# run-house/kubetorch

Hardware: NVIDIA H100
Metric: parallel_map_arg_plus_result_GBps (higher is better)
Workload: dtype f32

## Files before the change

### kubetorch_b200/csrc/ktb_dispatch.cu

```cuda
#include "ktb_common.cuh"

#include <algorithm>
#include <mutex>

namespace ktb {


constexpr int kBcastMax = 15;
constexpr int kBcastThreads = 256;
constexpr int kBcastUnroll = 2;

struct BcastDsts {
  uint8_t* d[kBcastMax];
  int n;
};

__global__ void __launch_bounds__(kBcastThreads)
    bcast_kernel(const uint8_t* src, const __grid_constant__ BcastDsts dsts, size_t n_bytes) {
  constexpr size_t VB = 32;
  constexpr size_t ROW = (size_t)kBcastThreads * VB;
  constexpr size_t TILE = ROW * kBcastUnroll;
  const size_t n_full = n_bytes / TILE;
  for (size_t t = blockIdx.x; t < n_full; t += gridDim.x) {
    const size_t off = t * TILE + (size_t)threadIdx.x * VB;
// ... 37 lines not shown
extern "C" {

int ktb_broadcast(int root, const void* src, void* const* dsts, int n_dst, size_t nbytes,
                  uintptr_t stream) {
  int rc = require_device(root);
  if (rc) return rc;
  KTB_REQUIRE(n_dst >= 0 && n_dst <= kBcastMax, KTB_ERR_ARG, "ktb_broadcast: n_dst %d out of range [0,%d]",
              n_dst, kBcastMax);
  if (nbytes == 0 || n_dst == 0) return KTB_OK;
  KTB_REQUIRE(src && dsts, KTB_ERR_ARG, "ktb_broadcast: null argument");
  BcastDsts b;
  b.n = 0;
  uintptr_t align = (uintptr_t)src;
  for (int k = 0; k < n_dst; ++k) {
    KTB_REQUIRE(dsts[k], KTB_ERR_ARG, "ktb_broadcast: dsts[%d] is null", k);
    if (dsts[k] == src) continue;
    b.d[b.n++] = static_cast<uint8_t*>(dsts[k]);
    align |= (uintptr_t)dsts[k];
  }
  if (b.n == 0) return KTB_OK;
  KTB_GUARD(root);
  const DeviceInfo* di = device_info(root);
  cudaStream_t st = reinterpret_cast<cudaStream_t>(stream);
  if ((align & 31) == 0) {
    size_t tiles = nbytes / ((size_t)kBcastThreads * 32 * kBcastUnroll);
    int grid = (int)std::min<size_t>(std::max<size_t>(tiles, 1), (size_t)di->sm_count * 4);
    bcast_kernel<<<grid, kBcastThreads, 0, st>>>(static_cast<const uint8_t*>(src), b, nbytes);
  } else {
    size_t blocks = (nbytes + 255) / 256;
    int grid = (int)std::min<size_t>(std::max<size_t>(blocks, 1), (size_t)di->sm_count * 8);
    bcast_bytes_kernel<<<grid, 256, 0, st>>>(static_cast<const uint8_t*>(src), b, nbytes);
  }
  KTB_CK(cudaGetLastError());
  return KTB_OK;
}

}

struct CallEvents {
  cudaEvent_t make(int device, int slot) {
    struct Pool {
      cudaEvent_t ev[kMaxDevices][kMaxDevices + 1] = {};
      ~Pool() {}
    };
    static thread_local Pool pool;
    if (device < 0 || device >= kMaxDevices || slot < 0 || slot > kMaxDevices) return nullptr;
    cudaEvent_t& e = pool.ev[device][slot];
    if (!e) {
      DeviceGuard g(device);
      if (!g.ok || cudaEventCreateWithFlags(&e, cudaEventDisableTiming) != cudaSuccess) {
        e = nullptr;
        return nullptr;
      }
    }
    return e;
  }
};

static int check_ranks(const char* who, int n_ranks, const int* devs, int root_rank) {
  KTB_REQUIRE(n_ranks > 0 && n_ranks <= kMaxDevices && devs, KTB_ERR_ARG, "%s: bad n_ranks %d", who, n_ranks);
  KTB_REQUIRE(root_rank >= 0 && root_rank < n_ranks, KTB_ERR_ARG, "%s: root_rank %d out of range", who, root_rank);
  for (int r = 0; r < n_ranks; ++r) {
    int rc = require_device(devs[r]);
    if (rc) return rc;
    if (devs[r] != devs[root_rank]) {
      KTB_REQUIRE(ktb_peer_enabled(devs[r], devs[root_rank]) == 1, KTB_ERR_UNSUPPORTED,
                  "%s: device %d has no peer access to root device %d", who, devs[r], devs[root_rank]);
    }
  }
  return KTB_OK;
}

static cudaStream_t rank_stream(const uintptr_t* streams, const int* devs, int r) {
  return streams ? reinterpret_cast<cudaStream_t>(streams[r]) : device_info(devs[r])->stream_rank;
}

template <class Launch>
static int fork_join(const char* who, size_t n_elems, size_t granule, int n_ranks, const int* devs, int root_rank,
                     const uintptr_t* streams, bool skip_empty, Launch&& launch) {
  const int root_dev = devs[root_rank];
  cudaStream_t root_stream = rank_stream(streams, devs, root_rank);
  CallEvents events;
  cudaEvent_t done[kMaxDevices] = {nullptr};
  cudaEvent_t args_ready = events.make(root_dev, 0);
  KTB_REQUIRE(args_ready, KTB_ERR_CUDA, "%s: cudaEventCreate failed", who);
  {
    KTB_GUARD(root_dev);
    KTB_CK(cudaEventRecord(args_ready, root_stream));
  }
  for (int r = 0; r < n_ranks; ++r) {
    size_t b = 0, e = 0;
    ktb_shard_bounds(n_elems / granule, n_ranks, r, &b, &e);
    b *= granule;
    e *= granule;
    if (skip_empty && e == b) continue;
    const int dev = devs[r];
    KTB_GUARD(dev);
    cudaStream_t st = rank_stream(streams, devs, r);
    const bool is_root = (r == root_rank) || (dev == root_dev && st == root_stream);
    if (!is_root) KTB_CK(cudaStreamWaitEvent(st, args_ready, 0));
    int rc = launch(r, dev, b, e, st);
    if (rc) return rc;
    if (!is_root) {
      done[r] = events.make(dev, 1 + r);
      KTB_REQUIRE(done[r], KTB_ERR_CUDA, "%s: cudaEventCreate failed", who);
      KTB_CK(cudaEventRecord(done[r], st));
    }
  }
  KTB_GUARD(root_dev);
  for (int r = 0; r < n_ranks; ++r)
    if (done[r]) KTB_CK(cudaStreamWaitEvent(root_stream, done[r], 0));
  return KTB_OK;
}

extern "C" {

int ktb_scatter_map_gather(int op, int dtype, const void* src_root, void* dst_root, size_t n_elems,
                           size_t granule, double alpha, double beta, int n_ranks, const int* devs,
                           int root_rank, int variant, const uintptr_t* streams) {
  int rc = check_ranks("ktb_scatter_map_gather", n_ranks, devs, root_rank);
  if (rc) return rc;
  const size_t es = dtype_size(dtype);
  KTB_REQUIRE(es != 0, KTB_ERR_ARG, "ktb_scatter_map_gather: unknown dtype %d", dtype);
  if (n_elems == 0) return KTB_OK;
  KTB_REQUIRE(src_root && dst_root, KTB_ERR_ARG, "ktb_scatter_map_gather: null src/dst");
  KTB_REQUIRE(granule > 0 && n_elems % granule == 0, KTB_ERR_ARG,
              "ktb_scatter_map_gather: n_elems %zu is not a multiple of granule %zu", n_elems, granule);
  const MapParams p = make_params(alpha, beta, dtype);
  return fork_join("ktb_scatter_map_gather", n_elems, granule, n_ranks, devs, root_rank, streams, true,
                   [&](int, int dev, size_t b, size_t e, cudaStream_t st) {
                     return launch_map(dev, op, dtype, static_cast<const uint8_t*>(src_root) + b * es,
                                       static_cast<uint8_t*>(dst_root) + b * es, e - b, p, variant, st);
                   });
}

int ktb_scatter_map_reduce(int op, int dtype, const void* src_root, size_t n_elems, size_t granule,
                           double alpha, double beta, int n_ranks, const int* devs, int root_rank,
                           void* partials_root, void* out_root, void* const* workspaces,
                           const uintptr_t* streams) {
  int rc = check_ranks("ktb_scatter_map_reduce", n_ranks, devs, root_rank);
  if (rc) return rc;
  const size_t es = dtype_size(dtype);
  KTB_REQUIRE(es != 0 && dtype != KTB_U8, KTB_ERR_ARG, "ktb_scatter_map_reduce: dtype %d not reducible", dtype);
  KTB_REQUIRE(partials_root && out_root && workspaces, KTB_ERR_ARG, "ktb_scatter_map_reduce: null argument");
  for (int r = 0; r < n_ranks; ++r)
    KTB_REQUIRE(workspaces[r], KTB_ERR_ARG, "ktb_scatter_map_reduce: workspaces[%d] is null", r);
  KTB_REQUIRE(src_root || n_elems == 0, KTB_ERR_ARG, "ktb_scatter_map_reduce: null src");
  KTB_REQUIRE(granule > 0 && n_elems % granule == 0, KTB_ERR_ARG,
              "ktb_scatter_map_reduce: n_elems %zu is not a multiple of granule %zu", n_elems, granule);
  const MapParams p = make_params(alpha, beta, dtype);
  const size_t acc_size = (dtype == KTB_F32 || dtype == KTB_BF16 || dtype == KTB_F16) ? 4 : 8;
  rc = fork_join("ktb_scatter_map_reduce", n_elems, granule, n_ranks, devs, root_rank, streams, false,
                 [&](int r, int dev, size_t b, size_t e, cudaStream_t st) {
                   return launch_map_reduce(dev, op, dtype, static_cast<const uint8_t*>(src_root) + b * es, e - b, p,
                                            static_cast<uint8_t*>(partials_root) + (size_t)r * acc_size,
                                            workspaces[r], st);
                 });
  if (rc) return rc;
  KTB_GUARD(devs[root_rank]);
  return launch_reduce_partials(devs[root_rank], dtype, partials_root, n_ranks, out_root,
                                rank_stream(streams, devs, root_rank));
}


}
```

### kubetorch_b200/csrc/ktb_map.cu

```cuda
#include "ktb_common.cuh"

#include <algorithm>
#include <atomic>

namespace ktb {

extern int g_red_ctas_per_sm;
extern int g_red_loads;
extern int g_red_fold;
extern int g_seg_large;
extern int g_mlp_chunk_rows;
}
extern int g_mlp_stage_ce;
namespace ktb {
extern std::atomic<int> g_host_zero_copy;
}
extern std::atomic<int> g_push_scatter_ctas_per_sm;
extern std::atomic<int> g_push_slice;
namespace ktb {

static std::atomic<int> g_vec_ctas_per_sm{0};
static std::atomic<int> g_tma_ctas_per_sm{1};
static std::atomic<int> g_tma_cfg{0};
static std::atomic<int> g_auto_variant{KTB_VARIANT_VEC};
static std::atomic<int> g_vec_flavor{2};
static std::atomic<int> g_vec_unroll{4};

constexpr int kVecThreads = 256;
constexpr int kVecUnroll = 4;
constexpr int kVecFlavor = 2;

template <int VB, int FL>
__device__ __forceinline__ void ld_vec(const uint8_t* p, uint32_t (&w)[VB / 4]) {
  static_assert(VB == 16, "sm_90 has no wider per-thread global access than 128 bits");
  if constexpr (FL == 1) {
    asm volatile("ld.global.v4.b32 {%0,%1,%2,%3}, [%4];"
                 : "=r"(w[0]), "=r"(w[1]), "=r"(w[2]), "=r"(w[3])
                 : "l"(p)
                 : "memory");
  } else if constexpr (FL == 2 || FL == 3) {
    ldg128_stream(p, w);
  } else {
    ldg128(p, w);
  }
}
template <int VB, int FL>
__device__ __forceinline__ void st_vec(uint8_t* p, const uint32_t (&w)[VB / 4]) {
  static_assert(VB == 16, "sm_90 has no wider per-thread global access than 128 bits");
  if constexpr (FL == 1) {
    asm volatile("st.global.v4.b32 [%0], {%1,%2,%3,%4};" ::"l"(p), "r"(w[0]), "r"(w[1]), "r"(w[2]), "r"(w[3])
                 : "memory");
  } else if constexpr (FL == 2) {
    stg128_stream(p, w);
  } else {
    stg128(p, w);
  }
}

template <int DT, int OP, int VB, int FL = kVecFlavor, int UNROLL = kVecUnroll>
__global__ void __launch_bounds__(kVecThreads)
    map_vec_kernel(const uint8_t* src, uint8_t* dst, size_t n_bytes, MapParams p) {
  constexpr int NW = VB / 4;
  constexpr int kVecUnroll = UNROLL;
  constexpr size_t TILE = (size_t)kVecThreads * kVecUnroll * VB;
  constexpr size_t ROW = (size_t)kVecThreads * VB;
  const size_t n_full = n_bytes / TILE;

  for (size_t t = blockIdx.x; t < n_full; t += gridDim.x) {
    const size_t off = t * TILE + (size_t)threadIdx.x * VB;
    uint32_t w[kVecUnroll][NW];
#pragma unroll
    for (int j = 0; j < kVecUnroll; ++j) ld_vec<VB, FL>(src + off + j * ROW, w[j]);
#pragma unroll
    for (int j = 0; j < kVecUnroll; ++j) {
      apply_words<DT, OP, NW>(w[j], p);
      st_vec<VB, FL>(dst + off + j * ROW, w[j]);
    }
  }

  if (blockIdx.x == (unsigned)(n_full % gridDim.x)) {
    const size_t base = n_full * TILE;
    const size_t n_vec = (n_bytes - base) / VB;
    for (size_t v = threadIdx.x; v < n_vec; v += kVecThreads) {
      uint32_t w[NW];
      ld_vec<VB, FL>(src + base + v * VB, w);
      apply_words<DT, OP, NW>(w, p);
      st_vec<VB, FL>(dst + base + v * VB, w);
    }
    constexpr size_t ES = (DT == KTB_U8) ? 1 : ((DT == KTB_BF16 || DT == KTB_F16) ? 2 : (DT == KTB_I64 ? 8 : 4));
    const size_t tail = base + n_vec * VB;
    const size_t n_tail = (n_bytes - tail) / ES;
    for (size_t e = threadIdx.x; e < n_tail; e += kVecThreads)
      apply_elem<DT, OP>(src + tail + e * ES, dst + tail + e * ES, p);
  }
}

template <int DT, int OP>
__global__ void __launch_bounds__(256)
    map_scalar_kernel(const uint8_t* src, uint8_t* dst, size_t n_elems, MapParams p) {
  constexpr size_t ES = (DT == KTB_U8) ? 1 : ((DT == KTB_BF16 || DT == KTB_F16) ? 2 : (DT == KTB_I64 ? 8 : 4));
  const size_t stride = (size_t)gridDim.x * blockDim.x;
  for (size_t i = (size_t)blockIdx.x * blockDim.x + threadIdx.x; i < n_elems; i += stride)
    apply_elem<DT, OP>(src + i * ES, dst + i * ES, p);
}

template <int DT, int OP, int STAGES, int STAGE_BYTES, int NT>
__global__ void __launch_bounds__(NT)
    map_tma_kernel(const uint8_t* src, uint8_t* dst, size_t n_bytes, MapParams p) {
  extern __shared__ __align__(128) uint8_t smem[];
  uint8_t* buf = smem;
  uint64_t* full = reinterpret_cast<uint64_t*>(smem + (size_t)STAGES * STAGE_BYTES);
  constexpr bool kCompute = !(OP == KTB_OP_IDENTITY || DT == KTB_U8);
// ... 246 lines not shown
```

### kubetorch_b200/csrc/ktb_mlp.cu

```cuda
#include "ktb_common.cuh"

#include <cuda.h>
#include <algorithm>
#include <atomic>
#include <climits>
#include <cmath>
#include <mutex>

namespace ktb {

constexpr int kMlpBlockM = 128;
constexpr int kMlpBlockK = 64;
constexpr int kMlpWgmmaK = 16;
constexpr int kMlpStages = 4;
constexpr int kMlpConsumers = 256;
constexpr int kMlpThreads = kMlpConsumers + 32;
int g_mlp_chunk_rows = 16896;

__device__ __forceinline__ void tma_load_2d(void* smem_dst, const CUtensorMap* map, int c0, int c1, uint64_t* bar) {
  asm volatile(
      "cp.async.bulk.tensor.2d.shared::cluster.global.mbarrier::complete_tx::bytes [%0], [%1, {%3, %4}], [%2];" ::
          "r"(smem_u32(smem_dst)),
      "l"(map), "r"(smem_u32(bar)), "r"(c0), "r"(c1)
      : "memory");
}
__device__ __forceinline__ void prefetch_tensormap(const CUtensorMap* map) {
  asm volatile("prefetch.tensormap [%0];" ::"l"(map) : "memory");
}
__device__ __forceinline__ void mbar_arrive(uint64_t* bar) {
  asm volatile("mbarrier.arrive.shared::cta.b64 _, [%0];" ::"r"(smem_u32(bar)) : "memory");
}
__device__ __forceinline__ void wgmma_fence() { asm volatile("wgmma.fence.sync.aligned;" ::: "memory"); }
__device__ __forceinline__ void wgmma_commit() { asm volatile("wgmma.commit_group.sync.aligned;" ::: "memory"); }
__device__ __forceinline__ void wgmma_wait_all() { asm volatile("wgmma.wait_group.sync.aligned 0;" ::: "memory"); }

__device__ __forceinline__ uint64_t make_smem_desc_sw128(const void* smem_tile) {
  const uint32_t addr = smem_u32(smem_tile);
  uint64_t d = 0;
  d |= (uint64_t)((addr & 0x3FFFFu) >> 4);
  d |= (uint64_t)1 << 16;
  d |= (uint64_t)(1024u >> 4) << 32;
  d |= (uint64_t)1 << 62;
  return d;
}

template <int N>
struct Wgmma;
template <>
struct Wgmma<256> {
  __device__ __forceinline__ static void mma(float (&d)[128], uint64_t adesc, uint64_t bdesc, uint32_t scale_d) {
    asm volatile(
        "{\n"
        ".reg .pred p;\n"
        "setp.ne.b32 p, %130, 0;\n"
        "wgmma.mma_async.sync.aligned.m64n256k16.f32.bf16.bf16 "
        "{%0,%1,%2,%3,%4,%5,%6,%7,%8,%9,%10,%11,%12,%13,%14,%15,%16,%17,%18,%19,%20,%21,%22,%23,%24,%25,%26,%27,%28,%29,%30,%31,%32,%33,%34,%35,%36,%37,%38,%39,%40,%41,%42,%43,%44,%45,%46,%47,%48,%49,%50,%51,%52,%53,%54,%55,%56,%57,%58,%59,%60,%61,%62,%63,%64,%65,%66,%67,%68,%69,%70,%71,%72,%73,%74,%75,%76,%77,%78,%79,%80,%81,%82,%83,%84,%85,%86,%87,%88,%89,%90,%91,%92,%93,%94,%95,%96,%97,%98,%99,%100,%101,%102,%103,%104,%105,%106,%107,%108,%109,%110,%111,%112,%113,%114,%115,%116,%117,%118,%119,%120,%121,%122,%123,%124,%125,%126,%127}, "
        "%128, %129, p, 1, 1, 0, 0;\n"
        "}\n"
        : "+f"(d[0]), "+f"(d[1]), "+f"(d[2]), "+f"(d[3]), "+f"(d[4]), "+f"(d[5]), "+f"(d[6]), "+f"(d[7]), "+f"(d[8]), "+f"(d[9]), "+f"(d[10]), "+f"(d[11]), "+f"(d[12]), "+f"(d[13]), "+f"(d[14]), "+f"(d[15]), "+f"(d[16]), "+f"(d[17]), "+f"(d[18]), "+f"(d[19]), "+f"(d[20]), "+f"(d[21]), "+f"(d[22]), "+f"(d[23]), "+f"(d[24]), "+f"(d[25]), "+f"(d[26]), "+f"(d[27]), "+f"(d[28]), "+f"(d[29]), "+f"(d[30]), "+f"(d[31]), "+f"(d[32]), "+f"(d[33]), "+f"(d[34]), "+f"(d[35]), "+f"(d[36]), "+f"(d[37]), "+f"(d[38]), "+f"(d[39]), "+f"(d[40]), "+f"(d[41]), "+f"(d[42]), "+f"(d[43]), "+f"(d[44]), "+f"(d[45]), "+f"(d[46]), "+f"(d[47]), "+f"(d[48]), "+f"(d[49]), "+f"(d[50]), "+f"(d[51]), "+f"(d[52]), "+f"(d[53]), "+f"(d[54]), "+f"(d[55]), "+f"(d[56]), "+f"(d[57]), "+f"(d[58]), "+f"(d[59]), "+f"(d[60]), "+f"(d[61]), "+f"(d[62]), "+f"(d[63]), "+f"(d[64]), "+f"(d[65]), "+f"(d[66]), "+f"(d[67]), "+f"(d[68]), "+f"(d[69]), "+f"(d[70]), "+f"(d[71]), "+f"(d[72]), "+f"(d[73]), "+f"(d[74]), "+f"(d[75]), "+f"(d[76]), "+f"(d[77]), "+f"(d[78]), "+f"(d[79]), "+f"(d[80]), "+f"(d[81]), "+f"(d[82]), "+f"(d[83]), "+f"(d[84]), "+f"(d[85]), "+f"(d[86]), "+f"(d[87]), "+f"(d[88]), "+f"(d[89]), "+f"(d[90]), "+f"(d[91]), "+f"(d[92]), "+f"(d[93]), "+f"(d[94]), "+f"(d[95]), "+f"(d[96]), "+f"(d[97]), "+f"(d[98]), "+f"(d[99]), "+f"(d[100]), "+f"(d[101]), "+f"(d[102]), "+f"(d[103]), "+f"(d[104]), "+f"(d[105]), "+f"(d[106]), "+f"(d[107]), "+f"(d[108]), "+f"(d[109]), "+f"(d[110]), "+f"(d[111]), "+f"(d[112]), "+f"(d[113]), "+f"(d[114]), "+f"(d[115]), "+f"(d[116]), "+f"(d[117]), "+f"(d[118]), "+f"(d[119]), "+f"(d[120]), "+f"(d[121]), "+f"(d[122]), "+f"(d[123]), "+f"(d[124]), "+f"(d[125]), "+f"(d[126]), "+f"(d[127])
        : "l"(adesc), "l"(bdesc), "r"(scale_d));
  }
};

template <>
struct Wgmma<128> {
  __device__ __forceinline__ static void mma(float (&d)[64], uint64_t adesc, uint64_t bdesc, uint32_t scale_d) {
    asm volatile(
        "{\n"
        ".reg .pred p;\n"
        "setp.ne.b32 p, %66, 0;\n"
        "wgmma.mma_async.sync.aligned.m64n128k16.f32.bf16.bf16 "
        "{%0,%1,%2,%3,%4,%5,%6,%7,%8,%9,%10,%11,%12,%13,%14,%15,%16,%17,%18,%19,%20,%21,%22,%23,%24,%25,%26,%27,%28,%29,%30,%31,%32,%33,%34,%35,%36,%37,%38,%39,%40,%41,%42,%43,%44,%45,%46,%47,%48,%49,%50,%51,%52,%53,%54,%55,%56,%57,%58,%59,%60,%61,%62,%63}, "
        "%64, %65, p, 1, 1, 0, 0;\n"
        "}\n"
        : "+f"(d[0]), "+f"(d[1]), "+f"(d[2]), "+f"(d[3]), "+f"(d[4]), "+f"(d[5]), "+f"(d[6]), "+f"(d[7]), "+f"(d[8]), "+f"(d[9]), "+f"(d[10]), "+f"(d[11]), "+f"(d[12]), "+f"(d[13]), "+f"(d[14]), "+f"(d[15]), "+f"(d[16]), "+f"(d[17]), "+f"(d[18]), "+f"(d[19]), "+f"(d[20]), "+f"(d[21]), "+f"(d[22]), "+f"(d[23]), "+f"(d[24]), "+f"(d[25]), "+f"(d[26]), "+f"(d[27]), "+f"(d[28]), "+f"(d[29]), "+f"(d[30]), "+f"(d[31]), "+f"(d[32]), "+f"(d[33]), "+f"(d[34]), "+f"(d[35]), "+f"(d[36]), "+f"(d[37]), "+f"(d[38]), "+f"(d[39]), "+f"(d[40]), "+f"(d[41]), "+f"(d[42]), "+f"(d[43]), "+f"(d[44]), "+f"(d[45]), "+f"(d[46]), "+f"(d[47]), "+f"(d[48]), "+f"(d[49]), "+f"(d[50]), "+f"(d[51]), "+f"(d[52]), "+f"(d[53]), "+f"(d[54]), "+f"(d[55]), "+f"(d[56]), "+f"(d[57]), "+f"(d[58]), "+f"(d[59]), "+f"(d[60]), "+f"(d[61]), "+f"(d[62]), "+f"(d[63])
        : "l"(adesc), "l"(bdesc), "r"(scale_d));
  }
};

template <>
struct Wgmma<64> {
  __device__ __forceinline__ static void mma(float (&d)[32], uint64_t adesc, uint64_t bdesc, uint32_t scale_d) {
    asm volatile(
        "{\n"
        ".reg .pred p;\n"
        "setp.ne.b32 p, %34, 0;\n"
        "wgmma.mma_async.sync.aligned.m64n64k16.f32.bf16.bf16 "
        "{%0,%1,%2,%3,%4,%5,%6,%7,%8,%9,%10,%11,%12,%13,%14,%15,%16,%17,%18,%19,%20,%21,%22,%23,%24,%25,%26,%27,%28,%29,%30,%31}, "
        "%32, %33, p, 1, 1, 0, 0;\n"
        "}\n"
        : "+f"(d[0]), "+f"(d[1]), "+f"(d[2]), "+f"(d[3]), "+f"(d[4]), "+f"(d[5]), "+f"(d[6]), "+f"(d[7]), "+f"(d[8]), "+f"(d[9]), "+f"(d[10]), "+f"(d[11]), "+f"(d[12]), "+f"(d[13]), "+f"(d[14]), "+f"(d[15]), "+f"(d[16]), "+f"(d[17]), "+f"(d[18]), "+f"(d[19]), "+f"(d[20]), "+f"(d[21]), "+f"(d[22]), "+f"(d[23]), "+f"(d[24]), "+f"(d[25]), "+f"(d[26]), "+f"(d[27]), "+f"(d[28]), "+f"(d[29]), "+f"(d[30]), "+f"(d[31])
        : "l"(adesc), "l"(bdesc), "r"(scale_d));
  }
};
template <int BLOCK_N, int STAGES>
struct MlpSmem {
  static constexpr int kABytes = kMlpBlockM * kMlpBlockK * 2;
  static constexpr int kBBytes = BLOCK_N * kMlpBlockK * 2;
  static constexpr int kStageBytes = kABytes + kBBytes;
  static constexpr int kBarrierOff = STAGES * kStageBytes;
  static constexpr int kTotal = kBarrierOff + 2 * STAGES * 8 + 1024 ;
};

template <int BLOCK_N, int STAGES>
__device__ __forceinline__ bool mlp_tile_mainloop(const CUtensorMap* map_a, const CUtensorMap* map_b, int K, int m0,
                                                  int n0, float (&acc)[BLOCK_N / 2]) {
  using S = MlpSmem<BLOCK_N, STAGES>;
  extern __shared__ uint8_t smem_raw[];
  uint8_t* smem = reinterpret_cast<uint8_t*>((reinterpret_cast<uintptr_t>(smem_raw) + 1023) & ~(uintptr_t)1023);
  uint64_t* full = reinterpret_cast<uint64_t*>(smem + S::kBarrierOff);
  uint64_t* empty = full + STAGES;

  const int warp = threadIdx.x >> 5;
  const int lane = threadIdx.x & 31;
  const int num_kb = K / kMlpBlockK;

  if (threadIdx.x == 0) {
#pragma unroll
    for (int s = 0; s < STAGES; ++s) {
      mbar_init(&full[s], 1);
      mbar_init(&empty[s], kMlpConsumers);
    }
    fence_barrier_init();
  }
  __syncthreads();

  if (warp == kMlpConsumers / 32) {
    if (lane == 0) {
      prefetch_tensormap(map_a);
      prefetch_tensormap(map_b);
      for (int kb = 0; kb < num_kb; ++kb) {
        const int s = kb % STAGES;
        mbar_wait(&empty[s], ((kb / STAGES) & 1) ^ 1);
        uint8_t* a_dst = smem + (size_t)s * S::kStageBytes;
        mbar_expect_tx(&full[s], S::kStageBytes);
        tma_load_2d(a_dst, map_a, kb * kMlpBlockK, m0, &full[s]);
        tma_load_2d(a_dst + S::kABytes, map_b, kb * kMlpBlockK, n0, &full[s]);
      }
    }
    return false;
  }

  const int wg = warp >> 2;
#pragma unroll
  for (int i = 0; i < BLOCK_N / 2; ++i) acc[i] = 0.f;
  for (int kb = 0; kb < num_kb; ++kb) {
    const int s = kb % STAGES;
    mbar_wait(&full[s], (kb / STAGES) & 1);
    const uint8_t* a_src = smem + (size_t)s * S::kStageBytes + wg * 64 * 128;
    const uint64_t adesc = make_smem_desc_sw128(a_src);
    const uint64_t bdesc = make_smem_desc_sw128(smem + (size_t)s * S::kStageBytes + S::kABytes);
    wgmma_fence();
#pragma unroll
    for (int k = 0; k < kMlpBlockK / kMlpWgmmaK; ++k) {
      Wgmma<BLOCK_N>::mma(acc, adesc + (uint64_t)(2 * k), bdesc + (uint64_t)(2 * k), (uint32_t)((kb | k) != 0));
    }
    wgmma_commit();
    wgmma_wait_all();
    mbar_arrive(&empty[s]);
  }
  return true;
}

__device__ __forceinline__ bool argmax_before(float v, int col, float best, int best_col) {
  const bool v_nan = v != v, best_nan = best != best;
  if (v_nan || best_nan) return v_nan && (!best_nan || col < best_col);
  return v > best || (v == best && col < best_col);
}

__device__ __forceinline__ uint4 philox4x32_10(uint4 c, uint2 k) {
#pragma unroll
  for (int i = 0; i < 10; ++i) {
    const uint32_t hi0 = __umulhi(0xD2511F53u, c.x), lo0 = 0xD2511F53u * c.x;
    const uint32_t hi1 = __umulhi(0xCD9E8D57u, c.z), lo1 = 0xCD9E8D57u * c.z;
    c = make_uint4(hi1 ^ c.y ^ k.x, lo1, hi0 ^ c.w ^ k.y, lo0);
    k.x += 0x9E3779B9u;
    k.y += 0xBB67AE85u;
  }
  return c;
}

__device__ __forceinline__ float gumbel_of(uint32_t x) {
  const float u = (float)(2u * (x >> 9) + 1u) * 5.9604644775390625e-8f;
  return -logf(-logf(u));
}

__device__ __forceinline__ void layer_pair(float a0, float a1, float a2, float a3, const __nv_bfloat16* bias, int col,
                                           int n_valid, int relu, __nv_bfloat162& y0, __nv_bfloat162& y1) {
  float v[4] = {a0, a1, a2, a3};
  if (bias != nullptr) {
#pragma unroll
    for (int c = 0; c < 2; ++c) {
      if (col + c < n_valid) {
        const float b = __bfloat162float(bias[col + c]);
        v[c] += b;
        v[2 + c] += b;
      }
    }
  }
  if (relu) {
#pragma unroll
    for (int q = 0; q < 4; ++q) v[q] = fmaxf(v[q], 0.f);
  }
  y0 = __floats2bfloat162_rn(v[0], v[1]);
  y1 = __floats2bfloat162_rn(v[2], v[3]);
}

template <int BLOCK_N>
__device__ __forceinline__ void sample_epilogue(const float (&acc)[BLOCK_N / 2], const __nv_bfloat16* bias, int col0,
                                                int n_valid, int relu, int row, bool st0, bool st1, int64_t* actions,
                                                float* log_probs, uint64_t seed, uint64_t row_base) {
  float mx[2] = {-INFINITY, -INFINITY};
  __nv_bfloat162 y[BLOCK_N / 4];
#pragma unroll
  for (int j = 0; j < BLOCK_N / 8; ++j) {
    const int col = col0 + 8 * j;
    if (col >= n_valid) continue;
    layer_pair(acc[4 * j], acc[4 * j + 1], acc[4 * j + 2], acc[4 * j + 3], bias, col, n_valid, relu, y[2 * j],
               y[2 * j + 1]);
#pragma unroll
    for (int q = 0; q < 4; ++q) {
      const float v = q & 1 ? __high2float(y[2 * j + (q >> 1)]) : __low2float(y[2 * j + (q >> 1)]);
      if (col + (q & 1) < n_valid && v > mx[q >> 1]) mx[q >> 1] = v;
    }
  }
#pragma unroll
  for (int h = 0; h < 2; ++h) {
#pragma unroll
    for (int m = 1; m <= 2; m <<= 1) {
      const float o = __shfl_xor_sync(0xffffffffu, mx[h], m);
      if (o > mx[h]) mx[h] = o;
    }
  }
  const uint2 key = make_uint2((uint32_t)seed, (uint32_t)(seed >> 32));
  float best[2] = {-INFINITY, -INFINITY}, best_y[2] = {0.f, 0.f}, sum[2] = {0.f, 0.f};
  int best_col[2] = {INT_MAX, INT_MAX};
#pragma unroll
  for (int j = 0; j < BLOCK_N / 8; ++j) {
    const int col = col0 + 8 * j;
    if (col >= n_valid) continue;
#pragma unroll
    for (int h = 0; h < 2; ++h) {
      const uint64_t i = row_base + (uint64_t)(row + 8 * h);
      const uint4 x = philox4x32_10(make_uint4((uint32_t)i, (uint32_t)(i >> 32), (uint32_t)col >> 1, 0u), key);
// ... 23 lines not shown
        best[h] = ov;
        best_col[h] = oc;
        best_y[h] = oy;
      }
    }
  }
  if ((threadIdx.x & 3) == 0) {
    if (st0) {
      actions[row] = best_col[0];
      log_probs[row] = best_y[0] - mx[0] - logf(sum[0]);
    }
    if (st1) {
      actions[row + 8] = best_col[1];
      log_probs[row + 8] = best_y[1] - mx[1] - logf(sum[1]);
    }
  }
}

template <int BLOCK_N, int STAGES>
__device__ __forceinline__ void gaussian_epilogue(const float (&acc)[BLOCK_N / 2], const __nv_bfloat16* bias, int col0,
                                                  int n_valid, int relu, int row, bool st0, bool st1,
                                                  const float* log_std, float* actions, float* log_probs,
                                                  uint64_t seed, uint64_t row_base) {
  asm volatile("" : "+l"(seed), "+l"(row_base), "+l"(bias), "+r"(col0), "+r"(n_valid), "+r"(row));
  using S = MlpSmem<BLOCK_N, STAGES>;
  static_assert(BLOCK_N / 64 <= STAGES, "each warp's bf16 pairs fill its 16 A rows of BLOCK_N / 64 stages");
  extern __shared__ uint8_t smem_raw[];
  uint8_t* smem = reinterpret_cast<uint8_t*>((reinterpret_cast<uintptr_t>(smem_raw) + 1023) & ~(uintptr_t)1023);
  uint8_t* mine = smem + (threadIdx.x >> 5) * 16 * 128 + (threadIdx.x & 31) * 4;
  auto slot = [&](int w) { return reinterpret_cast<__nv_bfloat162*>(mine + (w >> 4) * S::kStageBytes + (w & 15) * 128); };
#pragma unroll
  for (int j = 0; j < BLOCK_N / 8; ++j) {
    const int col = col0 + 8 * j;
    if (col >= n_valid) continue;
    layer_pair(acc[4 * j], acc[4 * j + 1], acc[4 * j + 2], acc[4 * j + 3], bias, col, n_valid, relu, *slot(2 * j),
               *slot(2 * j + 1));
  }
  const uint2 key = make_uint2((uint32_t)seed, (uint32_t)(seed >> 32));
  const bool pairs = (n_valid & 1) == 0 && ((uintptr_t)actions & 7) == 0;
  float sum[2] = {0.f, 0.f};
#pragma unroll 1
  for (int j = 0; j < BLOCK_N / 8; ++j) {
    const int col = col0 + 8 * j;
    if (col >= n_valid) break;
    const __nv_bfloat162 y[2] = {*slot(2 * j), *slot(2 * j + 1)};
    const bool has1 = col + 1 < n_valid;
    const float ls[2] = {log_std[col], has1 ? log_std[col + 1] : 0.f};
    const float sg[2] = {expf(ls[0]), expf(ls[1])};
#pragma unroll
    for (int h = 0; h < 2; ++h) {
      const uint64_t i = row_base + (uint64_t)(row + 8 * h);
      const uint4 x = philox4x32_10(make_uint4((uint32_t)i, (uint32_t)(i >> 32), (uint32_t)col >> 1, 1u), key);
      float a[2];
#pragma unroll
      for (int c = 0; c < 2; ++c) {
        const float u = (float)(2u * ((c ? x.y : x.x) >> 9) + 1u) * 5.9604644775390625e-8f;
        const float z = normcdfinvf(u);
        a[c] = __fadd_rn(c ? __high2float(y[h]) : __low2float(y[h]), __fmul_rn(sg[c], z));
        if (c == 0 || has1) sum[h] += 0.5f * z * z + ls[c];
      }
      if (!(h ? st1 : st0)) continue;
      float* p = actions + (size_t)(row + 8 * h) * n_valid + col;
      if (pairs) {
        *reinterpret_cast<float2*>(p) = make_float2(a[0], a[1]);
      } else {
        p[0] = a[0];
        if (has1) p[1] = a[1];
      }
    }
  }
#pragma unroll
  for (int h = 0; h < 2; ++h) {
#pragma unroll
    for (int m = 1; m <= 2; m <<= 1) sum[h] += __shfl_xor_sync(0xffffffffu, sum[h], m);
  }
  if ((threadIdx.x & 3) == 0) {
    const float c = (float)n_valid * 0.918938533204672742f;
    if (st0) log_probs[row] = -sum[0] - c;
    if (st1) log_probs[row + 8] = -sum[1] - c;
  }
}

template <int BLOCK_N, int STAGES>
__global__ void __launch_bounds__(kMlpThreads, 1)
    mlp_layer_wgmma_kernel(const __grid_constant__ CUtensorMap map_a, const __grid_constant__ CUtensorMap map_b,
                           const __nv_bfloat16* __restrict__ bias, __nv_bfloat16* __restrict__ C,
                           int64_t* __restrict__ actions, float* __restrict__ log_probs, uint64_t seed,
                           uint64_t row_base, const float* __restrict__ log_std, float* __restrict__ gauss_actions,
                           int ldc, int n_valid, int K, int rows, int relu) {
  const int n0 = blockIdx.x * BLOCK_N;
  const int m0 = blockIdx.y * kMlpBlockM;
  const int lane = threadIdx.x & 31;
  const int col0 = n0 + 2 * (lane & 3);
  float acc[BLOCK_N / 2];
  if (!mlp_tile_mainloop<BLOCK_N, STAGES>(&map_a, &map_b, K, m0, n0, acc)) return;
  const int warp = threadIdx.x >> 5;
  const int wg = warp >> 2;

  const int row = m0 + wg * 64 + (warp & 3) * 16 + (lane >> 2);
  const bool st0 = row < rows, st1 = row + 8 < rows;
  if (log_std != nullptr) {
    gaussian_epilogue<BLOCK_N, STAGES>(acc, bias, col0, n_valid, relu, row, st0, st1, log_std, gauss_actions,
                                       log_probs, seed, row_base);
    return;
  }
  if (log_probs != nullptr) {
    sample_epilogue<BLOCK_N>(acc, bias, col0, n_valid, relu, row, st0, st1, actions, log_probs, seed, row_base);
    return;
  }
  const bool pairs = C != nullptr && (ldc & 1) == 0 && ((uintptr_t)C & 3) == 0;
  if (pairs && actions == nullptr && n0 + BLOCK_N <= n_valid) {
    __nv_bfloat16* p0 = C + (size_t)row * ldc + col0;
    __nv_bfloat16* p1 = p0 + (size_t)8 * ldc;
#pragma unroll
    for (int j = 0; j < BLOCK_N / 8; ++j) {
      __nv_bfloat162 y0, y1;
      layer_pair(acc[4 * j], acc[4 * j + 1], acc[4 * j + 2], acc[4 * j + 3], bias, col0 + 8 * j, n_valid, relu, y0, y1);
      if (st0) *reinterpret_cast<__nv_bfloat162*>(p0 + 8 * j) = y0;
      if (st1) *reinterpret_cast<__nv_bfloat162*>(p1 + 8 * j) = y1;
    }
    return;
  }
  float best[2] = {-INFINITY, -INFINITY};
  int best_col[2] = {INT_MAX, INT_MAX};
#pragma unroll
  for (int j = 0; j < BLOCK_N / 8; ++j) {
    const int col = col0 + 8 * j;
    __nv_bfloat162 y0, y1;
    layer_pair(acc[4 * j], acc[4 * j + 1], acc[4 * j + 2], acc[4 * j + 3], bias, col, n_valid, relu, y0, y1);
    if (C != nullptr) {
      __nv_bfloat16* p0 = C + (size_t)row * ldc + col;
      __nv_bfloat16* p1 = p0 + (size_t)8 * ldc;
      if (pairs && col + 1 < n_valid) {
        if (st0) *reinterpret_cast<__nv_bfloat162*>(p0) = y0;
        if (st1) *reinterpret_cast<__nv_bfloat162*>(p1) = y1;
      } else {
        if (st0 && col < n_valid) p0[0] = y0.x;
        if (st1 && col < n_valid) p1[0] = y1.x;
        if (st0 && col + 1 < n_valid) p0[1] = y0.y;
        if (st1 && col + 1 < n_valid) p1[1] = y1.y;
      }
    }
    if (actions != nullptr) {
      const float r[4] = {__low2float(y0), __high2float(y0), __low2float(y1), __high2float(y1)};
#pragma unroll
      for (int q = 0; q < 4; ++q) {
        const int h = q >> 1, c = col + (q & 1);
        if (c < n_valid && argmax_before(r[q], c, best[h], best_col[h])) {
          best[h] = r[q];
          best_col[h] = c;
        }
      }
    }
  }
  if (actions != nullptr) {
#pragma unroll
    for (int h = 0; h < 2; ++h) {
#pragma unroll
      for (int m = 1; m <= 2; m <<= 1) {
        const float ov = __shfl_xor_sync(0xffffffffu, best[h], m);
        const int oc = __shfl_xor_sync(0xffffffffu, best_col[h], m);
        if (argmax_before(ov, oc, best[h], best_col[h])) {
          best[h] = ov;
          best_col[h] = oc;
        }
      }
    }
    if ((lane & 3) == 0) {
      if (st0) actions[row] = best_col[0];
      if (st1) actions[row + 8] = best_col[1];
    }
  }
}

typedef CUresult (*PFN_tensorMapEncodeTiled)(CUtensorMap*, CUtensorMapDataType, cuuint32_t, void*, const cuuint64_t*,
                                             const cuuint64_t*, const cuuint32_t*, const cuuint32_t*,
                                             CUtensorMapInterleave, CUtensorMapSwizzle, CUtensorMapL2promotion,
                                             CUtensorMapFloatOOBfill);
static PFN_tensorMapEncodeTiled g_encode = nullptr;
static std::once_flag g_encode_once;

static int get_encoder() {
  std::call_once(g_encode_once, [] {
    void* fn = nullptr;
    cudaDriverEntryPointQueryResult qres;
    if (cudaGetDriverEntryPoint("cuTensorMapEncodeTiled", &fn, cudaEnableDefault, &qres) == cudaSuccess &&
        qres == cudaDriverEntryPointSuccess)
      g_encode = reinterpret_cast<PFN_tensorMapEncodeTiled>(fn);
  });
  KTB_REQUIRE(g_encode != nullptr, KTB_ERR_CUDA, "cuTensorMapEncodeTiled is not available from the driver");
  return KTB_OK;
}

static int encode_map(CUtensorMap* map, const void* base, uint64_t rows, uint64_t cols, uint32_t box_rows);

static int make_map(CUtensorMap* map, const void* base, uint64_t rows, uint64_t cols, uint32_t box_rows) {
  struct Key {
    const void* base;
    uint64_t rows, cols;
    uint32_t box;
    bool operator==(const Key& o) const { return base == o.base && rows == o.rows && cols == o.cols && box == o.box; }
  };
  struct Slot {
    Key key;
    CUtensorMap map;
    bool used = false;
  };
  constexpr int kSlots = 64;
  thread_local Slot cache[kSlots];
  const Key k{base, rows, cols, box_rows};
  const size_t h = ((uintptr_t)base >> 8) * 0x9E3779B97F4A7C15ull + rows * 31 + cols * 7 + box_rows;
  Slot& s = cache[h % kSlots];
  if (s.used && s.key == k) {
    *map = s.map;
    return KTB_OK;
  }
  int rc = encode_map(map, base, rows, cols, box_rows);
  if (rc) return rc;
  s.key = k;
  s.map = *map;
  s.used = true;
  return KTB_OK;
}

static int encode_map(CUtensorMap* map, const void* base, uint64_t rows, uint64_t cols, uint32_t box_rows) {
  cuuint64_t gdim[2] = {cols, rows};
  cuuint64_t gstride[1] = {cols * 2};
  cuuint32_t box[2] = {(cuuint32_t)kMlpBlockK, box_rows};
  cuuint32_t estr[2] = {1, 1};
  CUresult r = g_encode(map, CU_TENSOR_MAP_DATA_TYPE_BFLOAT16, 2, const_cast<void*>(base), gdim, gstride, box, estr,
                        CU_TENSOR_MAP_INTERLEAVE_NONE, CU_TENSOR_MAP_SWIZZLE_128B, CU_TENSOR_MAP_L2_PROMOTION_L2_256B,
                        CU_TENSOR_MAP_FLOAT_OOB_FILL_NONE);
  KTB_REQUIRE(r == CUDA_SUCCESS, KTB_ERR_CUDA, "cuTensorMapEncodeTiled failed with CUresult %d", (int)r);
  return KTB_OK;
}

template <typename KernelT>
static int ensure_smem_attr(KernelT kfn, int smem_bytes, std::atomic<unsigned>& done_mask, int dev) {
  if (dev >= 0 && dev < 32 && (done_mask.load(std::memory_order_acquire) & (1u << dev))) return KTB_OK;
  cudaError_t e = cudaFuncSetAttribute(kfn, cudaFuncAttributeMaxDynamicSharedMemorySize, smem_bytes);
  if (e != cudaSuccess) {
    set_error("cudaFuncSetAttribute(max dynamic shared memory = %d) failed: %s", smem_bytes, cudaGetErrorString(e));
    return KTB_ERR_CUDA;
  }
  if (dev >= 0 && dev < 32) done_mask.fetch_or(1u << dev, std::memory_order_release);
  return KTB_OK;
}

template <int BLOCK_N>
static int launch_layer(int dev, const void* A, const void* B, const void* bias, void* C, int64_t* actions,
                        float* log_probs, uint64_t seed, uint64_t row_base, const float* log_std, float* gauss_actions,
                        size_t M, int N, int K, int ldc, bool relu, cudaStream_t stream) {
  using S = MlpSmem<BLOCK_N, kMlpStages>;
  static_assert(S::kTotal <= 232448, "the TMA ring must fit the 227 KiB a block may own");
  CUtensorMap ma, mb;
  int rc = make_map(&ma, A, M, (uint64_t)K, kMlpBlockM);
  if (rc) return rc;
  rc = make_map(&mb, B, (uint64_t)N, (uint64_t)K, BLOCK_N);
  if (rc) return rc;
  auto kfn = mlp_layer_wgmma_kernel<BLOCK_N, kMlpStages>;
  static std::atomic<unsigned> attr_done{0};
  rc = ensure_smem_attr(kfn, S::kTotal, attr_done, dev);
  if (rc) return rc;
  dim3 grid((unsigned)((N + BLOCK_N - 1) / BLOCK_N), (unsigned)((M + kMlpBlockM - 1) / kMlpBlockM));
  kfn<<<grid, kMlpThreads, S::kTotal, stream>>>(ma, mb, static_cast<const __nv_bfloat16*>(bias),
                                                static_cast<__nv_bfloat16*>(C), actions, log_probs, seed, row_base,
                                                log_std, gauss_actions, ldc, N, K, (int)M, relu);
  KTB_CK(cudaGetLastError());
  return KTB_OK;
}

struct MlpParams {
  const void *W1, *b1, *W2, *b2, *W3, *b3;
  void* logits;
  int64_t* actions;
  float* log_probs = nullptr;
  uint64_t seed = 0, row_base = 0;
  const float* log_std = nullptr;
  float* gauss_actions = nullptr;
};

static int mlp_hidden(int dev, const void* A, const void* W, const void* b, void* H, size_t rows, int d_hidden, int K,
                      cudaStream_t st) {
  return launch_layer<256>(dev, A, W, b, H, nullptr, nullptr, 0, 0, nullptr, nullptr, rows, d_hidden, K, d_hidden,
                           true, st);
}

static int mlp_head(int dev, const MlpParams& p, const void* h2, size_t r0, size_t rows, int d_hidden, int d_out,
                    cudaStream_t st) {
  void* y = p.logits ? static_cast<__nv_bfloat16*>(p.logits) + r0 * d_out : nullptr;
  int64_t* act = p.actions ? p.actions + r0 : nullptr;
  float* lp = p.log_probs ? p.log_probs + r0 : nullptr;
  float* ga = p.gauss_actions ? p.gauss_actions + r0 * d_out : nullptr;
  const uint64_t rb = p.row_base + r0;
  if (d_out <= 64)
    return launch_layer<64>(dev, h2, p.W3, p.b3, y, act, lp, p.seed, rb, p.log_std, ga, rows, d_out, d_hidden, d_out,
                            false, st);
  if (d_out <= 128)
    return launch_layer<128>(dev, h2, p.W3, p.b3, y, act, lp, p.seed, rb, p.log_std, ga, rows, d_out, d_hidden, d_out,
                             false, st);
  return launch_layer<256>(dev, h2, p.W3, p.b3, y, act, lp, p.seed, rb, p.log_std, ga, rows, d_out, d_hidden, d_out,
                           false, st);
}

static int mlp_check(const char* fn, size_t M, int d_in, int d_hidden, int d_out, const MlpParams& p, const void* obs,
                     const void* scratch, const void* stage) {
  KTB_REQUIRE(d_in > 0 && d_in % kMlpBlockK == 0, KTB_ERR_ARG, "%s: d_in=%d must be a multiple of 64", fn, d_in);
  KTB_REQUIRE(d_hidden > 0 && d_hidden % 256 == 0, KTB_ERR_ARG, "%s: d_hidden=%d must be a multiple of 256", fn,
              d_hidden);
  if (M > 0) {
    KTB_REQUIRE(p.logits || p.actions || p.log_std, KTB_ERR_ARG, "%s: logits and actions are both null", fn);
    if (p.log_std) {
      KTB_REQUIRE(p.gauss_actions && p.log_probs && !p.logits && !p.actions, KTB_ERR_ARG,
                  "%s: the Gaussian head needs fp32 actions and log_probs, and stores nothing else", fn);
      KTB_REQUIRE((((uintptr_t)p.log_std | (uintptr_t)p.gauss_actions) & 3) == 0, KTB_ERR_ARG,
                  "%s: log_std and actions must be 4-byte aligned", fn);
    }
    KTB_REQUIRE(d_out >= 1, KTB_ERR_ARG, "%s: d_out=%d must be positive", fn, d_out);
    KTB_REQUIRE(d_out <= 256, KTB_ERR_UNSUPPORTED, "%s: d_out=%d (heads up to 256 wide)", fn, d_out);
    KTB_REQUIRE((((uintptr_t)p.logits | (uintptr_t)p.b1 | (uintptr_t)p.b2 | (uintptr_t)p.b3) & 1) == 0, KTB_ERR_ARG,
                "%s: logits and biases must be 2-byte aligned", fn);
    KTB_REQUIRE(((uintptr_t)p.actions & 7) == 0, KTB_ERR_ARG, "%s: actions must be 8-byte aligned", fn);
    KTB_REQUIRE(((uintptr_t)p.log_probs & 3) == 0, KTB_ERR_ARG, "%s: log_probs must be 4-byte aligned", fn);
  }
  KTB_REQUIRE((((uintptr_t)obs | (uintptr_t)p.W1 | (uintptr_t)p.W2 | (uintptr_t)p.W3 | (uintptr_t)scratch |
                (uintptr_t)stage) & 15) == 0,
              KTB_ERR_ARG, "%s: obs, weights, scratch and stage must be 16-byte aligned", fn);
  return KTB_OK;
}
}

using namespace ktb;

extern "C" {

size_t ktb_mlp_scratch_bytes(size_t M, int d_hidden) {
  const size_t rows = std::min<size_t>(M, (size_t)g_mlp_chunk_rows);
  return 2 * rows * (size_t)d_hidden * 2;
}

size_t ktb_mlp_stage_bytes(size_t M, int d_in) {
  const size_t rows = std::min<size_t>(M, (size_t)g_mlp_chunk_rows);
  return 2 * rows * (size_t)d_in * 2;
}

int g_mlp_stage_ce = 0;

// ... 239 lines not shown
```

Baseline: 2868.

## Make MLP kernel persistent with warp-specialized producer, plus unroll and event tweaks

The MLP WGMMA kernel becomes persistent: the grid is capped at the SM count, and each block loops over tiles. A full producer warpgroup gives up registers with setmaxnreg while consumers take more, and consumers keep one WGMMA group in flight before releasing a stage. The vector map kernel's unroll drops from 4 to 2, and fork_join skips creating and recording the args-ready event when there is a single rank. These are unrelated changes; for a parallel-map bandwidth metric, only the unroll and event changes plausibly matter.

```diff
diff --git a/kubetorch_b200/csrc/ktb_dispatch.cu b/kubetorch_b200/csrc/ktb_dispatch.cu
--- a/kubetorch_b200/csrc/ktb_dispatch.cu
+++ b/kubetorch_b200/csrc/ktb_dispatch.cu
@@ -143,9 +143,10 @@
   cudaStream_t root_stream = rank_stream(streams, devs, root_rank);
   CallEvents events;
   cudaEvent_t done[kMaxDevices] = {nullptr};
-  cudaEvent_t args_ready = events.make(root_dev, 0);
-  KTB_REQUIRE(args_ready, KTB_ERR_CUDA, "%s: cudaEventCreate failed", who);
-  {
+  cudaEvent_t args_ready = nullptr;
+  if (n_ranks > 1) {
+    args_ready = events.make(root_dev, 0);
+    KTB_REQUIRE(args_ready, KTB_ERR_CUDA, "%s: cudaEventCreate failed", who);
     KTB_GUARD(root_dev);
     KTB_CK(cudaEventRecord(args_ready, root_stream));
   }
diff --git a/kubetorch_b200/csrc/ktb_map.cu b/kubetorch_b200/csrc/ktb_map.cu
--- a/kubetorch_b200/csrc/ktb_map.cu
+++ b/kubetorch_b200/csrc/ktb_map.cu
@@ -24,10 +24,10 @@
 static std::atomic<int> g_tma_cfg{0};
 static std::atomic<int> g_auto_variant{KTB_VARIANT_VEC};
 static std::atomic<int> g_vec_flavor{2};
-static std::atomic<int> g_vec_unroll{4};
+static std::atomic<int> g_vec_unroll{2};
 
 constexpr int kVecThreads = 256;
-constexpr int kVecUnroll = 4;
+constexpr int kVecUnroll = 2;
 constexpr int kVecFlavor = 2;
 
 template <int VB, int FL>
diff --git a/kubetorch_b200/csrc/ktb_mlp.cu b/kubetorch_b200/csrc/ktb_mlp.cu
--- a/kubetorch_b200/csrc/ktb_mlp.cu
+++ b/kubetorch_b200/csrc/ktb_mlp.cu
@@ -14,7 +14,9 @@
 constexpr int kMlpWgmmaK = 16;
 constexpr int kMlpStages = 4;
 constexpr int kMlpConsumers = 256;
-constexpr int kMlpThreads = kMlpConsumers + 32;
+constexpr int kMlpThreads = kMlpConsumers + 128;
+constexpr int kMlpProducerRegs = 40;
+constexpr int kMlpConsumerRegs = 232;
 int g_mlp_chunk_rows = 16896;
 
 __device__ __forceinline__ void tma_load_2d(void* smem_dst, const CUtensorMap* map, int c0, int c1, uint64_t* bar) {
@@ -33,6 +35,11 @@
 __device__ __forceinline__ void wgmma_fence() { asm volatile("wgmma.fence.sync.aligned;" ::: "memory"); }
 __device__ __forceinline__ void wgmma_commit() { asm volatile("wgmma.commit_group.sync.aligned;" ::: "memory"); }
 __device__ __forceinline__ void wgmma_wait_all() { asm volatile("wgmma.wait_group.sync.aligned 0;" ::: "memory"); }
+__device__ __forceinline__ void wgmma_wait_one() { asm volatile("wgmma.wait_group.sync.aligned 1;" ::: "memory"); }
+template <int N>
+__device__ __forceinline__ void setmaxnreg_dec() { asm volatile("setmaxnreg.dec.sync.aligned.u32 %0;" ::"n"(N)); }
+template <int N>
+__device__ __forceinline__ void setmaxnreg_inc() { asm volatile("setmaxnreg.inc.sync.aligned.u32 %0;" ::"n"(N)); }
 
 __device__ __forceinline__ uint64_t make_smem_desc_sw128(const void* smem_tile) {
   const uint32_t addr = smem_u32(smem_tile);
@@ -99,54 +106,42 @@
   static constexpr int kBBytes = BLOCK_N * kMlpBlockK * 2;
   static constexpr int kStageBytes = kABytes + kBBytes;
   static constexpr int kBarrierOff = STAGES * kStageBytes;
-  static constexpr int kTotal = kBarrierOff + 2 * STAGES * 8 + 1024 ;
+  static constexpr int kTotal = kBarrierOff + (2 * STAGES + 1) * 8 + 1024 ;
 };
 
+
 template <int BLOCK_N, int STAGES>
-__device__ __forceinline__ bool mlp_tile_mainloop(const CUtensorMap* map_a, const CUtensorMap* map_b, int K, int m0,
-                                                  int n0, float (&acc)[BLOCK_N / 2]) {
+__device__ __forceinline__ void mlp_produce(const CUtensorMap* map_a, const CUtensorMap* map_b, uint8_t* smem,
+                                            uint64_t* full, uint64_t* empty, uint64_t* epi_done, int num_kb,
+                                            int n_tiles_n, int tiles) {
   using S = MlpSmem<BLOCK_N, STAGES>;
-  extern __shared__ uint8_t smem_raw[];
-  uint8_t* smem = reinterpret_cast<uint8_t*>((reinterpret_cast<uintptr_t>(smem_raw) + 1023) & ~(uintptr_t)1023);
-  uint64_t* full = reinterpret_cast<uint64_t*>(smem + S::kBarrierOff);
-  uint64_t* empty = full + STAGES;
-
-  const int warp = threadIdx.x >> 5;
-  const int lane = threadIdx.x & 31;
-  const int num_kb = K / kMlpBlockK;
-
-  if (threadIdx.x == 0) {
-#pragma unroll
-    for (int s = 0; s < STAGES; ++s) {
-      mbar_init(&full[s], 1);
-      mbar_init(&empty[s], kMlpConsumers);
-    }
-    fence_barrier_init();
-  }
-  __syncthreads();
-
-  if (warp == kMlpConsumers / 32) {
-    if (lane == 0) {
-      prefetch_tensormap(map_a);
-      prefetch_tensormap(map_b);
-      for (int kb = 0; kb < num_kb; ++kb) {
-        const int s = kb % STAGES;
-        mbar_wait(&empty[s], ((kb / STAGES) & 1) ^ 1);
-        uint8_t* a_dst = smem + (size_t)s * S::kStageBytes;
-        mbar_expect_tx(&full[s], S::kStageBytes);
-        tma_load_2d(a_dst, map_a, kb * kMlpBlockK, m0, &full[s]);
-        tma_load_2d(a_dst + S::kABytes, map_b, kb * kMlpBlockK, n0, &full[s]);
-      }
-    }
-    return false;
-  }
-
-  const int wg = warp >> 2;
+  prefetch_tensormap(map_a);
+  prefetch_tensormap(map_b);
+  uint32_t it = 0, tile_no = 0;
+  for (int t = blockIdx.x; t < tiles; t += gridDim.x, ++tile_no) {
+    const int m0 = (t / n_tiles_n) * kMlpBlockM, n0 = (t % n_tiles_n) * BLOCK_N;
+    if (epi_done != nullptr && tile_no > 0) mbar_wait(epi_done, (tile_no - 1) & 1);
+    for (int kb = 0; kb < num_kb; ++kb, ++it) {
+      const uint32_t s = it % STAGES;
+      mbar_wait(&empty[s], ((it / STAGES) & 1) ^ 1);
+      uint8_t* a_dst = smem + (size_t)s * S::kStageBytes;
+      mbar_expect_tx(&full[s], S::kStageBytes);
+      tma_load_2d(a_dst, map_a, kb * kMlpBlockK, m0, &full[s]);
+      tma_load_2d(a_dst + S::kABytes, map_b, kb * kMlpBlockK, n0, &full[s]);
+    }
+  }
+}
+
+template <int BLOCK_N, int STAGES>
+__device__ __forceinline__ void mlp_tile_mma(const uint8_t* smem, uint64_t* full, uint64_t* empty, int num_kb,
+                                             uint32_t& it, float (&acc)[BLOCK_N / 2]) {
+  using S = MlpSmem<BLOCK_N, STAGES>;
+  const int wg = threadIdx.x >> 7;
 #pragma unroll
   for (int i = 0; i < BLOCK_N / 2; ++i) acc[i] = 0.f;
-  for (int kb = 0; kb < num_kb; ++kb) {
-    const int s = kb % STAGES;
-    mbar_wait(&full[s], (kb / STAGES) & 1);
+  for (int kb = 0; kb < num_kb; ++kb, ++it) {
+    const uint32_t s = it % STAGES;
+    mbar_wait(&full[s], (it / STAGES) & 1);
     const uint8_t* a_src = smem + (size_t)s * S::kStageBytes + wg * 64 * 128;
     const uint64_t adesc = make_smem_desc_sw128(a_src);
     const uint64_t bdesc = make_smem_desc_sw128(smem + (size_t)s * S::kStageBytes + S::kABytes);
@@ -156,10 +151,11 @@
       Wgmma<BLOCK_N>::mma(acc, adesc + (uint64_t)(2 * k), bdesc + (uint64_t)(2 * k), (uint32_t)((kb | k) != 0));
     }
     wgmma_commit();
-    wgmma_wait_all();
-    mbar_arrive(&empty[s]);
-  }
-  return true;
+    wgmma_wait_one();
+    if (kb > 0) mbar_arrive(&empty[(it - 1) % STAGES]);
+  }
+  wgmma_wait_all();
+  mbar_arrive(&empty[(it - 1) % STAGES]);
 }
 
 __device__ __forceinline__ bool argmax_before(float v, int col, float best, int best_col) {
@@ -349,18 +345,14 @@
 }
 
 template <int BLOCK_N, int STAGES>
-__global__ void __launch_bounds__(kMlpThreads, 1)
-    mlp_layer_wgmma_kernel(const __grid_constant__ CUtensorMap map_a, const __grid_constant__ CUtensorMap map_b,
-                           const __nv_bfloat16* __restrict__ bias, __nv_bfloat16* __restrict__ C,
-                           int64_t* __restrict__ actions, float* __restrict__ log_probs, uint64_t seed,
-                           uint64_t row_base, const float* __restrict__ log_std, float* __restrict__ gauss_actions,
-                           int ldc, int n_valid, int K, int rows, int relu) {
-  const int n0 = blockIdx.x * BLOCK_N;
-  const int m0 = blockIdx.y * kMlpBlockM;
+__device__ __forceinline__ void mlp_tile_epilogue(const float (&acc)[BLOCK_N / 2], int m0, int n0,
+                                                  const __nv_bfloat16* __restrict__ bias, __nv_bfloat16* __restrict__ C,
+                                                  int64_t* __restrict__ actions, float* __restrict__ log_probs,
+                                                  uint64_t seed, uint64_t row_base, const float* __restrict__ log_std,
+                                                  float* __restrict__ gauss_actions, int ldc, int n_valid, int rows,
+                                                  int relu) {
   const int lane = threadIdx.x & 31;
   const int col0 = n0 + 2 * (lane & 3);
-  float acc[BLOCK_N / 2];
-  if (!mlp_tile_mainloop<BLOCK_N, STAGES>(&map_a, &map_b, K, m0, n0, acc)) return;
   const int warp = threadIdx.x >> 5;
   const int wg = warp >> 2;
 
@@ -436,6 +428,56 @@
     if ((lane & 3) == 0) {
       if (st0) actions[row] = best_col[0];
       if (st1) actions[row + 8] = best_col[1];
+    }
+  }
+}
+
+template <int BLOCK_N, int STAGES>
+__global__ void __launch_bounds__(kMlpThreads, 1)
+    mlp_layer_wgmma_kernel(const __grid_constant__ CUtensorMap map_a, const __grid_constant__ CUtensorMap map_b,
+                           const __nv_bfloat16* __restrict__ bias, __nv_bfloat16* __restrict__ C,
+                           int64_t* __restrict__ actions, float* __restrict__ log_probs, uint64_t seed,
+                           uint64_t row_base, const float* __restrict__ log_std, float* __restrict__ gauss_actions,
+                           int ldc, int n_valid, int K, int rows, int relu) {
+  using S = MlpSmem<BLOCK_N, STAGES>;
+  extern __shared__ uint8_t smem_raw[];
+  uint8_t* smem = reinterpret_cast<uint8_t*>((reinterpret_cast<uintptr_t>(smem_raw) + 1023) & ~(uintptr_t)1023);
+  uint64_t* full = reinterpret_cast<uint64_t*>(smem + S::kBarrierOff);
+  uint64_t* empty = full + STAGES;
+  uint64_t* epi_done = empty + STAGES;
+  const int num_kb = K / kMlpBlockK;
+  const int n_tiles_n = (n_valid + BLOCK_N - 1) / BLOCK_N;
+  const int tiles = n_tiles_n * ((rows + kMlpBlockM - 1) / kMlpBlockM);
+
+  if (threadIdx.x == 0) {
+#pragma unroll
+    for (int s = 0; s < STAGES; ++s) {
+      mbar_init(&full[s], 1);
+      mbar_init(&empty[s], kMlpConsumers);
+    }
+    mbar_init(epi_done, kMlpConsumers);
+    fence_barrier_init();
+  }
+  __syncthreads();
+
+  if (threadIdx.x >= kMlpConsumers) {
+    setmaxnreg_dec<kMlpProducerRegs>();
+    if (threadIdx.x == kMlpConsumers)
+      mlp_produce<BLOCK_N, STAGES>(&map_a, &map_b, smem, full, empty, log_std != nullptr ? epi_done : nullptr, num_kb,
+                                   n_tiles_n, tiles);
+    return;
+  }
+  setmaxnreg_inc<kMlpConsumerRegs>();
+  uint32_t it = 0;
+  for (int t = blockIdx.x; t < tiles; t += gridDim.x) {
+    const int m0 = (t / n_tiles_n) * kMlpBlockM, n0 = (t % n_tiles_n) * BLOCK_N;
+    float acc[BLOCK_N / 2];
+    mlp_tile_mma<BLOCK_N, STAGES>(smem, full, empty, num_kb, it, acc);
+    mlp_tile_epilogue<BLOCK_N, STAGES>(acc, m0, n0, bias, C, actions, log_probs, seed, row_base, log_std,
+                                       gauss_actions, ldc, n_valid, rows, relu);
+    if (log_std != nullptr) {
+      fence_proxy_async_smem();
+      mbar_arrive(epi_done);
     }
   }
 }
@@ -529,7 +571,8 @@
   static std::atomic<unsigned> attr_done{0};
   rc = ensure_smem_attr(kfn, S::kTotal, attr_done, dev);
   if (rc) return rc;
-  dim3 grid((unsigned)((N + BLOCK_N - 1) / BLOCK_N), (unsigned)((M + kMlpBlockM - 1) / kMlpBlockM));
+  const size_t tiles = (size_t)((N + BLOCK_N - 1) / BLOCK_N) * ((M + kMlpBlockM - 1) / kMlpBlockM);
+  const unsigned grid = (unsigned)std::min<size_t>(tiles, (size_t)device_info(dev)->sm_count);
   kfn<<<grid, kMlpThreads, S::kTotal, stream>>>(ma, mb, static_cast<const __nv_bfloat16*>(bias),
                                                 static_cast<__nv_bfloat16*>(C), actions, log_probs, seed, row_base,
                                                 log_std, gauss_actions, ldc, N, K, (int)M, relu);
```

After: 2892, median of 6. No clear change (+0.8%).
